# CederGroupHub/chgnet

Hardware: NVIDIA H100
Metric: structures_per_sec_EFS (higher is better)
Workload: dtype f32

## Files before the change

chgnet_b200/csrc/gated_ws.cu:

```cuda
#include "gated_common.cuh"
#include "tc.cuh"

namespace chg {
namespace gated {
namespace {

constexpr int WS_THREADS = 512;
constexpr int TR = 128;
constexpr int HALF_BYTES = TR * 64 * 4;
constexpr int IMG_BYTES = 64 * 64 * 4;
constexpr int STRIP = 16;

struct WsSmem {
  static constexpr int IMG_OFF = 0;
  static constexpr int HS_OFF = 4 * IMG_BYTES;
  static constexpr int O_OFF = HS_OFF + 2 * HALF_BYTES;
  static constexpr int GIDX_OFF = O_OFF + HALF_BYTES;
  static constexpr int EIDX_OFF = GIDX_OFF + 2 * 3 * TR * 4;
  static constexpr int B2_OFF = EIDX_OFF + 4 * TR * 4;
  static constexpr int LN_OFF = B2_OFF + 128 * 4;
  static constexpr int TOTAL = LN_OFF + 256 * 4;
};

struct WsBars {
  uint64_t a_full[2], a_empty[2];
};

struct FusedArgs {
  const float* p_a;
  const float* p_b;
  const float* p_c;
  const float* wgt;
  const int32_t* idx0;
  const int32_t* idx1;
  const int32_t* idx2;
  const int32_t* ptr;
  int32_t n_rows, n_seg;
  const float* w2t;
  const float* b2;
  const float* ln;
  float* out;
  float* parts;
  float* save_pre;
  float* save_p;
};

__device__ __forceinline__ void prefetch_l2(const void* p) { asm volatile("prefetch.global.L2 [%0];" ::"l"(p)); }
__device__ __forceinline__ int swz(int r, int c) { return r * 256 + ((c ^ (r & 7)) << 4); }

__device__ __forceinline__ void build_image_ws(uint8_t* hi, uint8_t* lo, const float* __restrict__ src, int ld, int col0,
                                               int tid) {
  for (int i = tid; i < 4096; i += (int)blockDim.x) {
    const int kk = i >> 6, n = i & 63;
    uint32_t h, l;
    tc::split_tf32(__ldg(src + (size_t)kk * ld + col0 + n), h, l);
    const uint32_t off = tc::kmajor_offset(n, kk, 64);
    *reinterpret_cast<uint32_t*>(hi + off) = h;
    *reinterpret_cast<uint32_t*>(lo + off) = l;
  }
}

__device__ __forceinline__ float quad_sum(float v) {
  v += __shfl_xor_sync(0xffffffffu, v, 1);
  v += __shfl_xor_sync(0xffffffffu, v, 2);
  return v;
}
__device__ __forceinline__ void bias_ln_frag(float (&d)[32], const float* s_b2, const float* s_gamma, const float* s_beta,
                                             bool use_ln, float* save_rows, int row0, int n_rows) {
#pragma unroll
  for (int i = 0; i < 32; ++i) d[i] += s_b2[tc::frag_col(i)];
  if (save_rows != nullptr) {
#pragma unroll
    for (int i = 0; i < 32; i += 2) {
      const int g = row0 + tc::frag_row(i);
      if (g < n_rows) *reinterpret_cast<float2*>(save_rows + (size_t)g * 128 + tc::frag_col(i)) = make_float2(d[i], d[i + 1]);
    }
  }
  if (!use_ln) return;
#pragma unroll
  for (int h = 0; h < 2; ++h) {
    float s1 = 0.f;
#pragma unroll
    for (int i = 0; i < 32; ++i)
      if (((i >> 1) & 1) == h) s1 += d[i];
    const float mean = quad_sum(s1) * (1.f / 64.f);
    float s2 = 0.f;
#pragma unroll
    for (int i = 0; i < 32; ++i)
      if (((i >> 1) & 1) == h) s2 = fmaf(d[i] - mean, d[i] - mean, s2);
    const float rstd = 1.f / sqrtf(quad_sum(s2) * (1.f / 64.f) + LN_EPS);
#pragma unroll
    for (int i = 0; i < 32; ++i)
      if (((i >> 1) & 1) == h) d[i] = fmaf((d[i] - mean) * rstd, s_gamma[tc::frag_col(i)], s_beta[tc::frag_col(i)]);
  }
}

template <int MODE>
__global__ void __launch_bounds__(WS_THREADS, 1) gated_ws_fwd_kernel(const FusedArgs a) {
  extern __shared__ __align__(1024) uint8_t smem_raw[];
  uint8_t* s_img = smem_raw + WsSmem::IMG_OFF;
  uint8_t* s_hs = smem_raw + WsSmem::HS_OFF;
  uint8_t* s_o = smem_raw + WsSmem::O_OFF;
  int* s_gidx = reinterpret_cast<int*>(smem_raw + WsSmem::GIDX_OFF);
  int* s_eidx = reinterpret_cast<int*>(smem_raw + WsSmem::EIDX_OFF);
  float* s_b2 = reinterpret_cast<float*>(smem_raw + WsSmem::B2_OFF);
  float* s_ln = reinterpret_cast<float*>(smem_raw + WsSmem::LN_OFF);
  __shared__ __align__(8) WsBars bars;

  const int tid = threadIdx.x, warp = tid >> 5, lane = tid & 31;
  const bool use_ln = a.ln != nullptr;
  const int n_tiles = (a.n_rows + TR - 1) / TR;

  build_image_ws(s_img, s_img + IMG_BYTES, a.w2t, 128, 0, tid);
  build_image_ws(s_img + 2 * IMG_BYTES, s_img + 3 * IMG_BYTES, a.w2t, 128, 64, tid);
  if (tid < 128) s_b2[tid] = a.b2[tid];
  if (tid < 256) s_ln[tid] = use_ln ? a.ln[tid] : 0.f;
  if (tid == 0) {
    for (int i = 0; i < 2; ++i) {
      tc::mbar_init(&bars.a_full[i], 128);
      tc::mbar_init(&bars.a_empty[i], 256);
    }
    tc::mbar_fence_init();
  }
  tc::fence_async_smem();
  __syncthreads();

  if (warp >= 8) {
    const int half = (warp - 8) >> 2;
    const int gt = tid - 256 - half * 128;
    const int tx = gt & 15, ty = gt >> 4;
    int* gi = s_gidx + half * 3 * TR;
    uint8_t* stage = s_hs + half * HALF_BYTES;
    const int col = half * 64 + tx * 4;
    constexpr int PB = 4;
    int tl = 0;
    for (int tile = blockIdx.x; tile < n_tiles; tile += gridDim.x, ++tl) {
      const int base = tile * TR;
      {
        const int r = min(base + gt, a.n_rows - 1);
        gi[gt] = a.idx0[r];
        gi[TR + gt] = a.idx1[r];
        gi[2 * TR + gt] = a.idx2[r];
      }
      tc::wg_barrier(1 + half, 128);
      {
        const int nt = tile + gridDim.x;
        if (nt < n_tiles) {
          const int r = min(nt * TR + gt, a.n_rows - 1);
          const float* row = MODE == BOND ? a.p_c + (size_t)r * 128 + half * 64 : a.p_b + (size_t)__ldg(a.idx2 + r) * 128 + half * 64;
          prefetch_l2(row);
          prefetch_l2(row + 32);
        }
      }
#pragma unroll 1
      for (int b = 0; b < 16 / PB; ++b) {
        float4 v[PB];
#pragma unroll
        for (int i = 0; i < PB; ++i) {
          const int row = ty + 8 * (b * PB + i);
          const float* s0 = a.p_a + (size_t)gi[row] * 256 + col;
          const float* s1 = a.p_a + (size_t)gi[TR + row] * 256 + 128 + col;
          const float* s2 = a.p_b + (size_t)gi[2 * TR + row] * 128 + col;
          v[i] = ldg4(s0) + ldg4(s1) + ldg4(s2);
          if (MODE == BOND) v[i] = v[i] + ldg4(a.p_c + (size_t)min(base + row, a.n_rows - 1) * 128 + col);
        }
        if (b == 0) tc::mbar_wait(&bars.a_empty[half], (tl & 1) ^ 1);
#pragma unroll
        for (int i = 0; i < PB; ++i) {
          const int row = ty + 8 * (b * PB + i);
          if (a.save_pre != nullptr && base + row < a.n_rows) stg4(a.save_pre + (size_t)(base + row) * 128 + col, v[i]);
          *reinterpret_cast<float4*>(stage + swz(row, tx)) =
              make_float4(silu_f(v[i].x), silu_f(v[i].y), silu_f(v[i].z), silu_f(v[i].w));
        }
      }
      tc::wg_barrier(1 + half, 128);
      tc::mbar_arrive(&bars.a_full[half]);
    }
  } else {
    const int cw = warp >> 2;
    const int t = tid & 127;
    const int row0 = cw * 64;
    int* s_seg = s_eidx;
    int* s_wrow = s_eidx + TR;
    int* s_sa = s_eidx + 2 * TR;
    int* s_sb = s_eidx + 3 * TR;
    const uint32_t img = tc::smem_u32(s_img);
    int tl = 0;
    for (int tile = blockIdx.x; tile < n_tiles; tile += gridDim.x, ++tl) {
      const int base = tile * TR;
      {
        const int r = min(base + t, a.n_rows - 1);
        if (cw == 0) {
          const int seg = a.idx0[r];
          s_seg[t] = seg;
          s_sa[t] = __ldg(a.ptr + seg);
          s_sb[t] = __ldg(a.ptr + seg + 1);
        } else {
          const int wr = MODE == BOND ? a.idx1[r] : a.idx2[r];
          s_wrow[t] = wr;
          prefetch_l2(a.wgt + (size_t)wr * 64);
          prefetch_l2(a.wgt + (size_t)wr * 64 + 32);
        }
      }
      float dc[32], dg[32];
#pragma unroll
      for (int i = 0; i < 32; ++i) dc[i] = dg[i] = 0.f;
      tc::mbar_wait(&bars.a_full[0], tl & 1);
      tc::wg_gemm_k64<64>(dc, [&](int r, int k) { return *reinterpret_cast<const float*>(s_hs + swz(row0 + r, k >> 2) + (k & 3) * 4); },
                          img, img + IMG_BYTES, 2048);
      tc::mbar_arrive(&bars.a_empty[0]);
      tc::mbar_wait(&bars.a_full[1], tl & 1);
      tc::wg_gemm_k64<64>(dg, [&](int r, int k) { return *reinterpret_cast<const float*>(s_hs + HALF_BYTES + swz(row0 + r, k >> 2) + (k & 3) * 4); },
                          img + 2 * IMG_BYTES, img + 3 * IMG_BYTES, 2048);
      tc::mbar_arrive(&bars.a_empty[1]);
      float* save = a.save_p != nullptr ? a.save_p + (size_t)base * 128 : nullptr;
      bias_ln_frag(dc, s_b2, s_ln, s_ln + 64, use_ln, save, row0, a.n_rows - base);
      bias_ln_frag(dg, s_b2 + 64, s_ln + 128, s_ln + 192, use_ln, save != nullptr ? save + 64 : nullptr, row0, a.n_rows - base);
#pragma unroll
      for (int i = 0; i < 32; i += 2) {
        const int r = row0 + tc::frag_row(i), c = tc::frag_col(i);
        *reinterpret_cast<float2*>(s_o + swz(r, c >> 2) + (c & 3) * 4) =
            make_float2(silu_f(dc[i]) * sigmoid_f(dg[i]), silu_f(dc[i + 1]) * sigmoid_f(dg[i + 1]));
      }
      tc::wg_barrier(3, 256);

      const int strip_lo = base + warp * STRIP;
      const int strip_hi = min(strip_lo + STRIP, a.n_rows);
      if (strip_lo < a.n_rows) {
        float2 w[STRIP];
#pragma unroll
        for (int i = 0; i < STRIP; ++i) {
          const int rr = warp * STRIP + i;
          const float2 w0 = __ldg(reinterpret_cast<const float2*>(a.wgt + (size_t)s_wrow[rr] * 64) + lane);
          if (MODE == ATOM) {
            w[i] = w0;
          } else {
            const float2 wi = __ldg(reinterpret_cast<const float2*>(a.wgt + (size_t)s_seg[rr] * 64) + lane);
            w[i] = make_float2(wi.x * w0.x, wi.y * w0.y);
          }
        }
        float2 acc = make_float2(0.f, 0.f);
        int cur_row = warp * STRIP;
        auto emit = [&](int row0_, const float2& v) {
          const int seg = s_seg[row0_], sa = s_sa[row0_], sb = s_sb[row0_];
          float* dst;
          if (sa >= strip_lo && sb <= strip_hi) {
            dst = a.out + (size_t)seg * 64;
          } else {
            dst = a.parts + ((size_t)(strip_lo / STRIP) * 2 + (sa < strip_lo ? 0 : 1)) * 64;
          }
          *reinterpret_cast<float2*>(dst + lane * 2) = v;
        };
#pragma unroll
        for (int i = 0; i < STRIP; ++i) {
          const int rr = warp * STRIP + i;
          if (strip_lo + i < strip_hi) {
            if (s_seg[rr] != s_seg[cur_row]) {
              emit(cur_row, acc);
              cur_row = rr;
              acc = make_float2(0.f, 0.f);
            }
            const float2 o = *reinterpret_cast<const float2*>(s_o + swz(rr, lane >> 1) + (lane & 1) * 8);
            acc.x = fmaf(o.x, w[i].x, acc.x);
            acc.y = fmaf(o.y, w[i].y, acc.y);
          }
        }
        emit(cur_row, acc);
      }
      tc::wg_barrier(3, 256);
    }
  }
}

__global__ void seg_stitch_kernel(const int32_t* __restrict__ ptr, int n_seg, const float* __restrict__ parts,
                                  float* __restrict__ out) {
  const int idx = blockIdx.x * blockDim.x + threadIdx.x;
  const int s = idx >> 4, l = idx & 15;
  if (s >= n_seg) return;
  const int a = ptr[s], b = ptr[s + 1];
  if (a >= b) {
    stg4(out + (size_t)s * 64 + l * 4, make_float4(0.f, 0.f, 0.f, 0.f));
    return;
  }
  const int k0 = a / STRIP, k1 = (b - 1) / STRIP;
  if (k0 == k1) return;
  float4 acc = ldg4(parts + ((size_t)k0 * 2 + 1) * 64 + l * 4);
  for (int k = k0 + 1; k <= k1; ++k) acc = acc + ldg4(parts + ((size_t)k * 2) * 64 + l * 4);
  stg4(out + (size_t)s * 64 + l * 4, acc);
}

template <int MODE>
int launch_fused(const FusedArgs& a, cudaStream_t stream) {
  if (a.n_seg == 0) return CHG_OK;
  if (a.n_rows > 0) {
    static bool attr_set = false;
    if (!attr_set) {
      CHG_CUDA(cudaFuncSetAttribute(gated_ws_fwd_kernel<MODE>, cudaFuncAttributeMaxDynamicSharedMemorySize, WsSmem::TOTAL));
      attr_set = true;
    }
    const int n_tiles = (a.n_rows + TR - 1) / TR;
    gated_ws_fwd_kernel<MODE><<<min(n_tiles, sm_count()), WS_THREADS, WsSmem::TOTAL, stream>>>(a);
    cudaError_t e = cudaGetLastError();
    if (e != cudaSuccess) {
      set_error("gated_ws_fwd_kernel: launch failed: %s", cudaGetErrorString(e));
      return CHG_ERR_CUDA;
    }
    count_launch();
  }
  seg_stitch_kernel<<<(a.n_seg * 16 + 255) / 256, 256, 0, stream>>>(a.ptr, a.n_seg, a.parts, a.out);
  CHG_LAUNCH_END();
}

}

int atom_conv_fused_ws(const float* pcn, const float* pe, const float* wag, const int32_t* center, const int32_t* nbr,
                       const int32_t* d2u, const int32_t* ptr_c, int n_edges, int n_atoms, const float* w2t, const float* b2,
                       const float* ln, float* agg, float* save_p, float* parts, cudaStream_t stream) {
  FusedArgs a{pcn, pe, nullptr, wag, center, nbr, d2u, ptr_c, n_edges, n_atoms, w2t, b2, ln, agg, parts, nullptr, save_p};
  return launch_fused<ATOM>(a, stream);
}

int bond_conv_fused_ws(const float* pij, const float* px, const float* pa, const float* wbg, const int32_t* ang_atom,
                       const int32_t* ang_i, const int32_t* ang_j, const int32_t* ptr_i, int n_angles, int n_slots,
                       const float* w2t, const float* b2, const float* ln, float* agg, float* save_pre, float* save_p,
                       float* parts, cudaStream_t stream) {
  FusedArgs a{pij, px, pa, wbg, ang_i, ang_j, ang_atom, ptr_i, n_angles, n_slots, w2t, b2, ln, agg, parts, save_pre, save_p};
  return launch_fused<BOND>(a, stream);
}

}
}

using namespace chg;

extern "C" int64_t chg_gated_fused_workspace_floats(int32_t n_rows) {
  if (n_rows < 0) return -1;
  const int64_t msg = (int64_t)n_rows * 64, parts = ((int64_t)n_rows + 15) / 16 * 128;
  return (msg > parts ? msg : parts) + 64;
}

extern "C" int chg_atom_conv_fused(const float* pcn, const float* pe, const float* wag, const int32_t* center,
                                   const int32_t* nbr, const int32_t* d2u, const int32_t* ptr_c, int32_t n_edges,
                                   int32_t n_atoms, const float* w2t, const float* b2, const float* ln, float* agg,
                                   float* save_p, float* work, void* stream) {
  CHG_CHECK_ARG(n_edges >= 0 && n_atoms >= 0, "negative size");
  if (n_atoms == 0) return CHG_OK;
  CHG_CHECK_ARG(ptr_c && agg, "null pointer");
  CHG_CHECK_ARG(n_edges == 0 || (pcn && pe && wag && center && nbr && d2u && w2t && b2 && work), "null pointer");
  if (gated_impl() == 3 && n_edges >= ws_min_rows())
    return gated::atom_conv_fused_ws(pcn, pe, wag, center, nbr, d2u, ptr_c, n_edges, n_atoms, w2t, b2, ln, agg, save_p, work,
                                     as_stream(stream));
  const int rc = chg_atom_conv_fwd(pcn, pe, wag, center, nbr, d2u, n_edges, w2t, b2, ln, work, save_p, nullptr, stream);
  if (rc != CHG_OK) return rc;
  return chg_segment_sum(work, 64, nullptr, ptr_c, n_atoms, n_edges, 0, agg, 64, stream);
}

extern "C" int chg_bond_conv_fused(const float* pij, const float* px, const float* pa, const float* wbg,
                                   const int32_t* ang_atom, const int32_t* ang_i, const int32_t* ang_j,
                                   const int32_t* ptr_i, int32_t n_angles, int32_t n_slots, const float* w2t,
                                   const float* b2, const float* ln, float* agg, float* save_pre, float* save_p,
                                   float* work, void* stream) {
  CHG_CHECK_ARG(n_angles >= 0 && n_slots >= 0, "negative size");
  if (n_slots == 0) return CHG_OK;
  CHG_CHECK_ARG(ptr_i && agg, "null pointer");
  CHG_CHECK_ARG(n_angles == 0 || (pij && px && pa && wbg && ang_atom && ang_i && ang_j && w2t && b2 && work), "null pointer");
  if (gated_impl() == 3 && n_angles >= ws_min_rows())
    return gated::bond_conv_fused_ws(pij, px, pa, wbg, ang_atom, ang_i, ang_j, ptr_i, n_angles, n_slots, w2t, b2, ln, agg,
                                     save_pre, save_p, work, as_stream(stream));
  const int rc = chg_bond_conv_fwd(pij, px, pa, wbg, ang_atom, ang_i, ang_j, n_angles, w2t, b2, ln, work, save_pre, save_p, stream);
  if (rc != CHG_OK) return rc;
  return chg_segment_sum(work, 64, nullptr, ptr_i, n_slots, n_angles, 0, agg, 64, stream);
}

namespace chg {
namespace gated {
namespace {

struct WsBwdSmem {
  static constexpr int IMG_OFF = 0;
  static constexpr int T1_OFF = 4 * IMG_BYTES;
  static constexpr int T2_OFF = T1_OFF + 2 * HALF_BYTES;
  static constexpr int PIDX_OFF = T2_OFF + 2 * HALF_BYTES;
  static constexpr int FIDX_OFF = PIDX_OFF + 3 * TR * 4;
  static constexpr int LN_OFF = FIDX_OFF + 3 * TR * 4;
  static constexpr int TOTAL = LN_OFF + 256 * 4;
};

struct WsBwdBars {
  uint64_t a_full, a_empty;
};

template <int MODE>
__global__ void __launch_bounds__(WS_THREADS, 1) gated_ws_bwd_kernel(const BwdArgs a) {
  extern __shared__ __align__(1024) uint8_t smem_raw[];
  uint8_t* s_img = smem_raw + WsBwdSmem::IMG_OFF;
  uint8_t* s_t1 = smem_raw + WsBwdSmem::T1_OFF;
  uint8_t* s_t2 = smem_raw + WsBwdSmem::T2_OFF;
  int* s_pidx = reinterpret_cast<int*>(smem_raw + WsBwdSmem::PIDX_OFF);
  int* s_fidx = reinterpret_cast<int*>(smem_raw + WsBwdSmem::FIDX_OFF);
  float* s_ln = reinterpret_cast<float*>(smem_raw + WsBwdSmem::LN_OFF);
  __shared__ __align__(8) WsBwdBars bars;

  const int tid = threadIdx.x, warp = tid >> 5;
  const bool use_ln = a.ln != nullptr;
  const int n_tiles = (a.n_rows + TR - 1) / TR;

  build_image_ws(s_img, s_img + IMG_BYTES, a.w2, 64, 0, tid);
  build_image_ws(s_img + 2 * IMG_BYTES, s_img + 3 * IMG_BYTES, a.w2 + 64 * 64, 64, 0, tid);
  if (tid < 256) s_ln[tid] = use_ln ? a.ln[tid] : 0.f;
  if (tid == 0) {
    tc::mbar_init(&bars.a_full, 256);
    tc::mbar_init(&bars.a_empty, 256);
    tc::mbar_fence_init();
  }
  tc::fence_async_smem();
  __syncthreads();

  if (warp < 8) {
    const int t = tid;
    const int tx = t & 15, ty = t >> 4;
    const int c0 = tx * 4;
    int tl = 0;
    for (int tile = blockIdx.x; tile < n_tiles; tile += gridDim.x, ++tl) {
      const int base = tile * TR;
      if (t < TR) {
        const int r = min(base + t, a.n_rows - 1);
        s_pidx[t] = a.idx0[r];
        s_pidx[TR + t] = a.idx1[r];
        if (MODE == ATOM) s_pidx[2 * TR + t] = a.idx2[r];
      }
      tc::wg_barrier(1, 256);
      {
        const int nt = tile + gridDim.x;
        if (nt < n_tiles) {
          const int r = min(nt * TR + (t & 127), a.n_rows - 1);
          const float* row = a.save_p + (size_t)r * 128 + (t >> 7) * 64;
          prefetch_l2(row);
          prefetch_l2(row + 32);
        }
      }
      float4 g1, g2, b1, b2v;
      if (use_ln) {
        g1 = lds4(s_ln + c0);
        b1 = lds4(s_ln + 64 + c0);
        g2 = lds4(s_ln + 128 + c0);
        b2v = lds4(s_ln + 192 + c0);
      }
      tc::mbar_wait(&bars.a_empty, (tl & 1) ^ 1);
#pragma unroll 2
      for (int pass = 0; pass < 8; ++pass) {
        const int row = pass * 16 + ty;
        const int g = base + row;
        const bool valid = g < a.n_rows;
        const int r = min(g, a.n_rows - 1);
        const float4 pc4 = ldg4(a.save_p + (size_t)r * 128 + c0);
        const float4 pg4 = ldg4(a.save_p + (size_t)r * 128 + 64 + c0);
        float4 gm, wv;
        if (MODE == ATOM) {
          gm = ldg4(a.g_in + (size_t)s_pidx[row] * 64 + c0);
          wv = ldg4(a.wgt + (size_t)s_pidx[2 * TR + row] * 64 + c0);
        } else {
          gm = ldg4(a.g_in + (size_t)s_pidx[row] * 64 + c0);
          wv = ldg4(a.wgt + (size_t)s_pidx[row] * 64 + c0);
        }
        float y1[4] = {pc4.x, pc4.y, pc4.z, pc4.w};
        float y2[4] = {pg4.x, pg4.y, pg4.z, pg4.w};
        float xh1[4], xh2[4], rstd1 = 1.f, rstd2 = 1.f;
        if (use_ln) {
          ln_stats(y1, xh1, rstd1);
          ln_stats(y2, xh2, rstd2);
#pragma unroll
          for (int j = 0; j < 4; ++j) {
            y1[j] = fmaf(xh1[j], f4at(g1, j), f4at(b1, j));
            y2[j] = fmaf(xh2[j], f4at(g2, j), f4at(b2v, j));
          }
        }
        float s1[4], core[4], gate[4];
        float4 o;
#pragma unroll
        for (int j = 0; j < 4; ++j) {
          s1[j] = sigmoid_f(y1[j]);
          core[j] = y1[j] * s1[j];
          gate[j] = sigmoid_f(y2[j]);
          f4at(o, j) = core[j] * gate[j];
        }
        float4 go;
        if (MODE == ATOM) {
          if (valid) stg4(a.g_w0 + (size_t)g * 64 + c0, gm * o);
          go = gm * wv;
        } else {
          const float4 wj = ldg4(a.wgt + (size_t)s_pidx[TR + row] * 64 + c0);
          const float4 gmo = gm * o;
          if (valid) {
            stg4(a.g_w0 + (size_t)g * 64 + c0, gmo * wj);
            stg4(a.g_w1 + (size_t)g * 64 + c0, gmo * wv);
          }
          go = gm * wv * wj;
        }
        float gy1[4], gy2[4];
#pragma unroll
        for (int j = 0; j < 4; ++j) {
          const float gj = f4at(go, j);
          gy1[j] = gj * gate[j] * (s1[j] * fmaf(y1[j], 1.f - s1[j], 1.f));
          gy2[j] = gj * core[j] * gate[j] * (1.f - gate[j]);
        }
        if (use_ln) {
          float gx[4], sa = 0.f, sb = 0.f;
#pragma unroll
          for (int j = 0; j < 4; ++j) {
            gx[j] = gy1[j] * f4at(g1, j);
            sa += gx[j];
            sb = fmaf(gx[j], xh1[j], sb);
          }
          sa = sum16(sa) * (1.f / 64.f);
          sb = sum16(sb) * (1.f / 64.f);
#pragma unroll
          for (int j = 0; j < 4; ++j) gy1[j] = rstd1 * (gx[j] - sa - xh1[j] * sb);
          sa = 0.f, sb = 0.f;
#pragma unroll
          for (int j = 0; j < 4; ++j) {
            gx[j] = gy2[j] * f4at(g2, j);
            sa += gx[j];
            sb = fmaf(gx[j], xh2[j], sb);
          }
          sa = sum16(sa) * (1.f / 64.f);
          sb = sum16(sb) * (1.f / 64.f);
#pragma unroll
          for (int j = 0; j < 4; ++j) gy2[j] = rstd2 * (gx[j] - sa - xh2[j] * sb);
        }
        *reinterpret_cast<float4*>(s_t1 + swz(row, tx)) = make_float4(gy1[0], gy1[1], gy1[2], gy1[3]);
        *reinterpret_cast<float4*>(s_t1 + HALF_BYTES + swz(row, tx)) = make_float4(gy2[0], gy2[1], gy2[2], gy2[3]);
      }
      tc::wg_barrier(1, 256);
      tc::mbar_arrive(&bars.a_full);
    }
  } else {
    const int t = tid - 256;
    const int tx = t & 15, ty = t >> 4;
    const int c0 = tx * 4;
    const int crow = t & 127, chalf = t >> 7;
    const int row0 = ((warp - 8) >> 2) * 64;
    const uint32_t img = tc::smem_u32(s_img);
    int tl = 0;
    for (int tile = blockIdx.x; tile < n_tiles; tile += gridDim.x, ++tl) {
      const int base = tile * TR;
      if (MODE == ATOM && t < TR) {
        const int r = min(base + t, a.n_rows - 1);
        s_fidx[t] = a.idx0[r];
        s_fidx[TR + t] = a.idx1[r];
        s_fidx[2 * TR + t] = a.idx2[r];
      }
      {
        const int r = min(base + crow, a.n_rows - 1);
        const float* row = MODE == ATOM ? a.p_b + (size_t)__ldg(a.idx2 + r) * 128 + chalf * 64 : a.save_pre + (size_t)r * 128 + chalf * 64;
        prefetch_l2(row);
        prefetch_l2(row + 32);
      }
      tc::mbar_wait(&bars.a_full, tl & 1);
#pragma unroll 1
      for (int half = 0; half < 2; ++half) {
        float d[32];
#pragma unroll
        for (int i = 0; i < 32; ++i) d[i] = 0.f;
        const uint8_t* src = s_t1 + half * HALF_BYTES;
        tc::wg_gemm_k64<64>(d, [&](int r, int k) { return *reinterpret_cast<const float*>(src + swz(row0 + r, k >> 2) + (k & 3) * 4); },
                            img + half * 2 * IMG_BYTES, img + (half * 2 + 1) * IMG_BYTES, 2048);
        uint8_t* dst = s_t2 + half * HALF_BYTES;
#pragma unroll
        for (int i = 0; i < 32; i += 2) {
          const int r = row0 + tc::frag_row(i), c = tc::frag_col(i);
          *reinterpret_cast<float2*>(dst + swz(r, c >> 2) + (c & 3) * 4) = make_float2(d[i], d[i + 1]);
        }
      }
      tc::mbar_arrive(&bars.a_empty);
      tc::wg_barrier(2, 256);
#pragma unroll 2
      for (int pass = 0; pass < 8; ++pass) {
        const int row = pass * 16 + ty;
        const int g = base + row;
        float4 vc, vg;
        if (MODE == ATOM) {
          const float* s0 = a.p_a + (size_t)s_fidx[row] * 256 + c0;
          const float* s1 = a.p_a + (size_t)s_fidx[TR + row] * 256 + 128 + c0;
          const float* s2 = a.p_b + (size_t)s_fidx[2 * TR + row] * 128 + c0;
          vc = ldg4(s0) + ldg4(s1) + ldg4(s2);
          vg = ldg4(s0 + 64) + ldg4(s1 + 64) + ldg4(s2 + 64);
        } else {
          const int r = min(g, a.n_rows - 1);
          vc = ldg4(a.save_pre + (size_t)r * 128 + c0);
          vg = ldg4(a.save_pre + (size_t)r * 128 + 64 + c0);
        }
        const float4 hc = *reinterpret_cast<const float4*>(s_t2 + swz(row, tx));
        const float4 hg = *reinterpret_cast<const float4*>(s_t2 + HALF_BYTES + swz(row, tx));
        if (g < a.n_rows) {
          stg4(a.g_pre + (size_t)g * 128 + c0,
               make_float4(hc.x * dsilu_f(vc.x), hc.y * dsilu_f(vc.y), hc.z * dsilu_f(vc.z), hc.w * dsilu_f(vc.w)));
          stg4(a.g_pre + (size_t)g * 128 + 64 + c0,
               make_float4(hg.x * dsilu_f(vg.x), hg.y * dsilu_f(vg.y), hg.z * dsilu_f(vg.z), hg.w * dsilu_f(vg.w)));
        }
      }
      tc::wg_barrier(2, 256);
    }
  }
}

template <int MODE>
int launch_ws_bwd(const BwdArgs& a, cudaStream_t stream) {
  if (a.n_rows == 0) return CHG_OK;
  static bool attr_set = false;
  if (!attr_set) {
    CHG_CUDA(cudaFuncSetAttribute(gated_ws_bwd_kernel<MODE>, cudaFuncAttributeMaxDynamicSharedMemorySize, WsBwdSmem::TOTAL));
    attr_set = true;
  }
  const int n_tiles = (a.n_rows + TR - 1) / TR;
  gated_ws_bwd_kernel<MODE><<<min(n_tiles, sm_count()), WS_THREADS, WsBwdSmem::TOTAL, stream>>>(a);
  CHG_LAUNCH_END();
}

}

int atom_conv_bwd_ws(const BwdArgs& a, cudaStream_t stream) { return launch_ws_bwd<ATOM>(a, stream); }
int bond_conv_bwd_ws(const BwdArgs& a, cudaStream_t stream) { return launch_ws_bwd<BOND>(a, stream); }

}
}
```

Measured before the change: 10910.

## Add L2 eviction-policy hints, bulk prefetches, and split backward empty barrier

```diff
diff --git a/chgnet_b200/csrc/gated_ws.cu b/chgnet_b200/csrc/gated_ws.cu
--- a/chgnet_b200/csrc/gated_ws.cu
+++ b/chgnet_b200/csrc/gated_ws.cu
@@ -46,6 +46,45 @@
 };
 
 __device__ __forceinline__ void prefetch_l2(const void* p) { asm volatile("prefetch.global.L2 [%0];" ::"l"(p)); }
+
+__device__ __forceinline__ uint64_t l2_evict_first() {
+  uint64_t p;
+  asm volatile("createpolicy.fractional.L2::evict_first.b64 %0, 1.0;" : "=l"(p));
+  return p;
+}
+__device__ __forceinline__ uint64_t l2_evict_last() {
+  uint64_t p;
+  asm volatile("createpolicy.fractional.L2::evict_last.b64 %0, 1.0;" : "=l"(p));
+  return p;
+}
+__device__ __forceinline__ float4 ldg4_stream(const float* p, uint64_t pol) {
+  float4 v;
+  asm("ld.global.nc.L1::no_allocate.L2::cache_hint.v4.f32 {%0, %1, %2, %3}, [%4], %5;"
+      : "=f"(v.x), "=f"(v.y), "=f"(v.z), "=f"(v.w) : "l"(p), "l"(pol));
+  return v;
+}
+__device__ __forceinline__ float4 ldg4_table(const float* p, uint64_t pol) {
+  float4 v;
+  asm("ld.global.nc.L2::cache_hint.v4.f32 {%0, %1, %2, %3}, [%4], %5;"
+      : "=f"(v.x), "=f"(v.y), "=f"(v.z), "=f"(v.w) : "l"(p), "l"(pol));
+  return v;
+}
+__device__ __forceinline__ float2 ldg2_table(const float* p, uint64_t pol) {
+  float2 v;
+  asm("ld.global.nc.L2::cache_hint.v2.f32 {%0, %1}, [%2], %3;" : "=f"(v.x), "=f"(v.y) : "l"(p), "l"(pol));
+  return v;
+}
+__device__ __forceinline__ void stg4_stream(float* p, const float4& v, uint64_t pol) {
+  asm volatile("st.global.L2::cache_hint.v4.f32 [%0], {%1, %2, %3, %4}, %5;" ::"l"(p), "f"(v.x), "f"(v.y), "f"(v.z), "f"(v.w),
+               "l"(pol)
+               : "memory");
+}
+__device__ __forceinline__ void stg2_stream(float* p, const float2& v, uint64_t pol) {
+  asm volatile("st.global.L2::cache_hint.v2.f32 [%0], {%1, %2}, %3;" ::"l"(p), "f"(v.x), "f"(v.y), "l"(pol) : "memory");
+}
+__device__ __forceinline__ void prefetch_half_row(const float* p, uint64_t pol) {
+  asm volatile("cp.async.bulk.prefetch.L2.global.L2::cache_hint [%0], 256, %1;" ::"l"(p), "l"(pol) : "memory");
+}
 __device__ __forceinline__ int swz(int r, int c) { return r * 256 + ((c ^ (r & 7)) << 4); }
 
 __device__ __forceinline__ void build_image_ws(uint8_t* hi, uint8_t* lo, const float* __restrict__ src, int ld, int col0,
@@ -66,14 +105,14 @@
   return v;
 }
 __device__ __forceinline__ void bias_ln_frag(float (&d)[32], const float* s_b2, const float* s_gamma, const float* s_beta,
-                                             bool use_ln, float* save_rows, int row0, int n_rows) {
+                                             bool use_ln, float* save_rows, int row0, int n_rows, uint64_t pol_stream) {
 #pragma unroll
   for (int i = 0; i < 32; ++i) d[i] += s_b2[tc::frag_col(i)];
   if (save_rows != nullptr) {
 #pragma unroll
     for (int i = 0; i < 32; i += 2) {
       const int g = row0 + tc::frag_row(i);
-      if (g < n_rows) *reinterpret_cast<float2*>(save_rows + (size_t)g * 128 + tc::frag_col(i)) = make_float2(d[i], d[i + 1]);
+      if (g < n_rows) stg2_stream(save_rows + (size_t)g * 128 + tc::frag_col(i), make_float2(d[i], d[i + 1]), pol_stream);
     }
   }
   if (!use_ln) return;
@@ -133,6 +172,7 @@
     uint8_t* stage = s_hs + half * HALF_BYTES;
     const int col = half * 64 + tx * 4;
     constexpr int PB = 4;
+    const uint64_t pol_stream = l2_evict_first(), pol_table = l2_evict_last();
     int tl = 0;
     for (int tile = blockIdx.x; tile < n_tiles; tile += gridDim.x, ++tl) {
       const int base = tile * TR;
@@ -147,9 +187,8 @@
         const int nt = tile + gridDim.x;
         if (nt < n_tiles) {
           const int r = min(nt * TR + gt, a.n_rows - 1);
-          const float* row = MODE == BOND ? a.p_c + (size_t)r * 128 + half * 64 : a.p_b + (size_t)__ldg(a.idx2 + r) * 128 + half * 64;
-          prefetch_l2(row);
-          prefetch_l2(row + 32);
+          if (MODE == BOND) prefetch_half_row(a.p_c + (size_t)r * 128 + half * 64, pol_stream);
+          else prefetch_half_row(a.p_b + (size_t)__ldg(a.idx2 + r) * 128 + half * 64, pol_table);
         }
       }
 #pragma unroll 1
@@ -161,14 +200,14 @@
           const float* s0 = a.p_a + (size_t)gi[row] * 256 + col;
           const float* s1 = a.p_a + (size_t)gi[TR + row] * 256 + 128 + col;
           const float* s2 = a.p_b + (size_t)gi[2 * TR + row] * 128 + col;
-          v[i] = ldg4(s0) + ldg4(s1) + ldg4(s2);
-          if (MODE == BOND) v[i] = v[i] + ldg4(a.p_c + (size_t)min(base + row, a.n_rows - 1) * 128 + col);
+          v[i] = ldg4_table(s0, pol_table) + ldg4_table(s1, pol_table) + ldg4_table(s2, pol_table);
+          if (MODE == BOND) v[i] = v[i] + ldg4_stream(a.p_c + (size_t)min(base + row, a.n_rows - 1) * 128 + col, pol_stream);
         }
         if (b == 0) tc::mbar_wait(&bars.a_empty[half], (tl & 1) ^ 1);
 #pragma unroll
         for (int i = 0; i < PB; ++i) {
           const int row = ty + 8 * (b * PB + i);
-          if (a.save_pre != nullptr && base + row < a.n_rows) stg4(a.save_pre + (size_t)(base + row) * 128 + col, v[i]);
+          if (a.save_pre != nullptr && base + row < a.n_rows) stg4_stream(a.save_pre + (size_t)(base + row) * 128 + col, v[i], pol_stream);
           *reinterpret_cast<float4*>(stage + swz(row, tx)) =
               make_float4(silu_f(v[i].x), silu_f(v[i].y), silu_f(v[i].z), silu_f(v[i].w));
         }
@@ -198,8 +237,7 @@
         } else {
           const int wr = MODE == BOND ? a.idx1[r] : a.idx2[r];
           s_wrow[t] = wr;
-          prefetch_l2(a.wgt + (size_t)wr * 64);
-          prefetch_l2(a.wgt + (size_t)wr * 64 + 32);
+          prefetch_half_row(a.wgt + (size_t)wr * 64, l2_evict_last());
         }
       }
       float dc[32], dg[32];
@@ -214,8 +252,10 @@
                           img + 2 * IMG_BYTES, img + 3 * IMG_BYTES, 2048);
       tc::mbar_arrive(&bars.a_empty[1]);
       float* save = a.save_p != nullptr ? a.save_p + (size_t)base * 128 : nullptr;
-      bias_ln_frag(dc, s_b2, s_ln, s_ln + 64, use_ln, save, row0, a.n_rows - base);
-      bias_ln_frag(dg, s_b2 + 64, s_ln + 128, s_ln + 192, use_ln, save != nullptr ? save + 64 : nullptr, row0, a.n_rows - base);
+      const uint64_t pol_stream = l2_evict_first();
+      bias_ln_frag(dc, s_b2, s_ln, s_ln + 64, use_ln, save, row0, a.n_rows - base, pol_stream);
+      bias_ln_frag(dg, s_b2 + 64, s_ln + 128, s_ln + 192, use_ln, save != nullptr ? save + 64 : nullptr, row0, a.n_rows - base,
+                   pol_stream);
 #pragma unroll
       for (int i = 0; i < 32; i += 2) {
         const int r = row0 + tc::frag_row(i), c = tc::frag_col(i);
@@ -227,15 +267,16 @@
       const int strip_lo = base + warp * STRIP;
       const int strip_hi = min(strip_lo + STRIP, a.n_rows);
       if (strip_lo < a.n_rows) {
+        const uint64_t pol_table = l2_evict_last();
         float2 w[STRIP];
 #pragma unroll
         for (int i = 0; i < STRIP; ++i) {
           const int rr = warp * STRIP + i;
-          const float2 w0 = __ldg(reinterpret_cast<const float2*>(a.wgt + (size_t)s_wrow[rr] * 64) + lane);
+          const float2 w0 = ldg2_table(a.wgt + (size_t)s_wrow[rr] * 64 + lane * 2, pol_table);
           if (MODE == ATOM) {
             w[i] = w0;
           } else {
-            const float2 wi = __ldg(reinterpret_cast<const float2*>(a.wgt + (size_t)s_seg[rr] * 64) + lane);
+            const float2 wi = ldg2_table(a.wgt + (size_t)s_seg[rr] * 64 + lane * 2, pol_table);
             w[i] = make_float2(wi.x * w0.x, wi.y * w0.y);
           }
         }
@@ -387,7 +428,7 @@
 };
 
 struct WsBwdBars {
-  uint64_t a_full, a_empty;
+  uint64_t a_full, a_empty[2];
 };
 
 template <int MODE>
@@ -410,7 +451,8 @@
   if (tid < 256) s_ln[tid] = use_ln ? a.ln[tid] : 0.f;
   if (tid == 0) {
     tc::mbar_init(&bars.a_full, 256);
-    tc::mbar_init(&bars.a_empty, 256);
+    tc::mbar_init(&bars.a_empty[0], 256);
+    tc::mbar_init(&bars.a_empty[1], 256);
     tc::mbar_fence_init();
   }
   tc::fence_async_smem();
@@ -420,9 +462,11 @@
     const int t = tid;
     const int tx = t & 15, ty = t >> 4;
     const int c0 = tx * 4;
+    const uint64_t pol_stream = l2_evict_first(), pol_table = l2_evict_last();
     int tl = 0;
     for (int tile = blockIdx.x; tile < n_tiles; tile += gridDim.x, ++tl) {
       const int base = tile * TR;
+      const int nt = tile + gridDim.x;
       if (t < TR) {
         const int r = min(base + t, a.n_rows - 1);
         s_pidx[t] = a.idx0[r];
@@ -430,15 +474,7 @@
         if (MODE == ATOM) s_pidx[2 * TR + t] = a.idx2[r];
       }
       tc::wg_barrier(1, 256);
-      {
-        const int nt = tile + gridDim.x;
-        if (nt < n_tiles) {
-          const int r = min(nt * TR + (t & 127), a.n_rows - 1);
-          const float* row = a.save_p + (size_t)r * 128 + (t >> 7) * 64;
-          prefetch_l2(row);
-          prefetch_l2(row + 32);
-        }
-      }
+      if (nt < n_tiles) prefetch_half_row(a.save_p + (size_t)min(nt * TR + (t & 127), a.n_rows - 1) * 128 + (t >> 7) * 64, pol_stream);
       float4 g1, g2, b1, b2v;
       if (use_ln) {
         g1 = lds4(s_ln + c0);
@@ -446,22 +482,21 @@
         g2 = lds4(s_ln + 128 + c0);
         b2v = lds4(s_ln + 192 + c0);
       }
-      tc::mbar_wait(&bars.a_empty, (tl & 1) ^ 1);
 #pragma unroll 2
       for (int pass = 0; pass < 8; ++pass) {
         const int row = pass * 16 + ty;
         const int g = base + row;
         const bool valid = g < a.n_rows;
         const int r = min(g, a.n_rows - 1);
-        const float4 pc4 = ldg4(a.save_p + (size_t)r * 128 + c0);
-        const float4 pg4 = ldg4(a.save_p + (size_t)r * 128 + 64 + c0);
+        const float4 pc4 = ldg4_stream(a.save_p + (size_t)r * 128 + c0, pol_stream);
+        const float4 pg4 = ldg4_stream(a.save_p + (size_t)r * 128 + 64 + c0, pol_stream);
         float4 gm, wv;
         if (MODE == ATOM) {
-          gm = ldg4(a.g_in + (size_t)s_pidx[row] * 64 + c0);
-          wv = ldg4(a.wgt + (size_t)s_pidx[2 * TR + row] * 64 + c0);
+          gm = ldg4_table(a.g_in + (size_t)s_pidx[row] * 64 + c0, pol_table);
+          wv = ldg4_table(a.wgt + (size_t)s_pidx[2 * TR + row] * 64 + c0, pol_table);
         } else {
-          gm = ldg4(a.g_in + (size_t)s_pidx[row] * 64 + c0);
-          wv = ldg4(a.wgt + (size_t)s_pidx[row] * 64 + c0);
+          gm = ldg4_table(a.g_in + (size_t)s_pidx[row] * 64 + c0, pol_table);
+          wv = ldg4_table(a.wgt + (size_t)s_pidx[row] * 64 + c0, pol_table);
         }
         float y1[4] = {pc4.x, pc4.y, pc4.z, pc4.w};
         float y2[4] = {pg4.x, pg4.y, pg4.z, pg4.w};
@@ -486,14 +521,14 @@
         }
         float4 go;
         if (MODE == ATOM) {
-          if (valid) stg4(a.g_w0 + (size_t)g * 64 + c0, gm * o);
+          if (valid) stg4_stream(a.g_w0 + (size_t)g * 64 + c0, gm * o, pol_stream);
           go = gm * wv;
         } else {
-          const float4 wj = ldg4(a.wgt + (size_t)s_pidx[TR + row] * 64 + c0);
+          const float4 wj = ldg4_table(a.wgt + (size_t)s_pidx[TR + row] * 64 + c0, pol_table);
           const float4 gmo = gm * o;
           if (valid) {
-            stg4(a.g_w0 + (size_t)g * 64 + c0, gmo * wj);
-            stg4(a.g_w1 + (size_t)g * 64 + c0, gmo * wv);
+            stg4_stream(a.g_w0 + (size_t)g * 64 + c0, gmo * wj, pol_stream);
+            stg4_stream(a.g_w1 + (size_t)g * 64 + c0, gmo * wv, pol_stream);
           }
           go = gm * wv * wj;
         }
@@ -528,7 +563,9 @@
 #pragma unroll
           for (int j = 0; j < 4; ++j) gy2[j] = rstd2 * (gx[j] - sa - xh2[j] * sb);
         }
+        if (pass == 0) tc::mbar_wait(&bars.a_empty[0], (tl & 1) ^ 1);
         *reinterpret_cast<float4*>(s_t1 + swz(row, tx)) = make_float4(gy1[0], gy1[1], gy1[2], gy1[3]);
+        if (pass == 0) tc::mbar_wait(&bars.a_empty[1], (tl & 1) ^ 1);
         *reinterpret_cast<float4*>(s_t1 + HALF_BYTES + swz(row, tx)) = make_float4(gy2[0], gy2[1], gy2[2], gy2[3]);
       }
       tc::wg_barrier(1, 256);
@@ -541,6 +578,7 @@
     const int crow = t & 127, chalf = t >> 7;
     const int row0 = ((warp - 8) >> 2) * 64;
     const uint32_t img = tc::smem_u32(s_img);
+    const uint64_t pol_stream = l2_evict_first(), pol_table = l2_evict_last();
     int tl = 0;
     for (int tile = blockIdx.x; tile < n_tiles; tile += gridDim.x, ++tl) {
       const int base = tile * TR;
@@ -552,9 +590,8 @@
       }
       {
         const int r = min(base + crow, a.n_rows - 1);
-        const float* row = MODE == ATOM ? a.p_b + (size_t)__ldg(a.idx2 + r) * 128 + chalf * 64 : a.save_pre + (size_t)r * 128 + chalf * 64;
-        prefetch_l2(row);
-        prefetch_l2(row + 32);
+        if (MODE == ATOM) prefetch_half_row(a.p_b + (size_t)__ldg(a.idx2 + r) * 128 + chalf * 64, pol_table);
+        else prefetch_half_row(a.save_pre + (size_t)r * 128 + chalf * 64, pol_stream);
       }
       tc::mbar_wait(&bars.a_full, tl & 1);
 #pragma unroll 1
@@ -565,6 +602,7 @@
         const uint8_t* src = s_t1 + half * HALF_BYTES;
         tc::wg_gemm_k64<64>(d, [&](int r, int k) { return *reinterpret_cast<const float*>(src + swz(row0 + r, k >> 2) + (k & 3) * 4); },
                             img + half * 2 * IMG_BYTES, img + (half * 2 + 1) * IMG_BYTES, 2048);
+        tc::mbar_arrive(&bars.a_empty[half]);
         uint8_t* dst = s_t2 + half * HALF_BYTES;
 #pragma unroll
         for (int i = 0; i < 32; i += 2) {
@@ -572,7 +610,6 @@
           *reinterpret_cast<float2*>(dst + swz(r, c >> 2) + (c & 3) * 4) = make_float2(d[i], d[i + 1]);
         }
       }
-      tc::mbar_arrive(&bars.a_empty);
       tc::wg_barrier(2, 256);
 #pragma unroll 2
       for (int pass = 0; pass < 8; ++pass) {
@@ -583,20 +620,20 @@
           const float* s0 = a.p_a + (size_t)s_fidx[row] * 256 + c0;
           const float* s1 = a.p_a + (size_t)s_fidx[TR + row] * 256 + 128 + c0;
           const float* s2 = a.p_b + (size_t)s_fidx[2 * TR + row] * 128 + c0;
-          vc = ldg4(s0) + ldg4(s1) + ldg4(s2);
-          vg = ldg4(s0 + 64) + ldg4(s1 + 64) + ldg4(s2 + 64);
+          vc = ldg4_table(s0, pol_table) + ldg4_table(s1, pol_table) + ldg4_table(s2, pol_table);
+          vg = ldg4_table(s0 + 64, pol_table) + ldg4_table(s1 + 64, pol_table) + ldg4_table(s2 + 64, pol_table);
         } else {
           const int r = min(g, a.n_rows - 1);
-          vc = ldg4(a.save_pre + (size_t)r * 128 + c0);
-          vg = ldg4(a.save_pre + (size_t)r * 128 + 64 + c0);
+          vc = ldg4_stream(a.save_pre + (size_t)r * 128 + c0, pol_stream);
+          vg = ldg4_stream(a.save_pre + (size_t)r * 128 + 64 + c0, pol_stream);
         }
         const float4 hc = *reinterpret_cast<const float4*>(s_t2 + swz(row, tx));
         const float4 hg = *reinterpret_cast<const float4*>(s_t2 + HALF_BYTES + swz(row, tx));
         if (g < a.n_rows) {
-          stg4(a.g_pre + (size_t)g * 128 + c0,
-               make_float4(hc.x * dsilu_f(vc.x), hc.y * dsilu_f(vc.y), hc.z * dsilu_f(vc.z), hc.w * dsilu_f(vc.w)));
-          stg4(a.g_pre + (size_t)g * 128 + 64 + c0,
-               make_float4(hg.x * dsilu_f(vg.x), hg.y * dsilu_f(vg.y), hg.z * dsilu_f(vg.z), hg.w * dsilu_f(vg.w)));
+          stg4_stream(a.g_pre + (size_t)g * 128 + c0,
+                      make_float4(hc.x * dsilu_f(vc.x), hc.y * dsilu_f(vc.y), hc.z * dsilu_f(vc.z), hc.w * dsilu_f(vc.w)), pol_stream);
+          stg4_stream(a.g_pre + (size_t)g * 128 + 64 + c0,
+                      make_float4(hg.x * dsilu_f(vg.x), hg.y * dsilu_f(vg.y), hg.z * dsilu_f(vg.z), hg.w * dsilu_f(vg.w)), pol_stream);
         }
       }
       tc::wg_barrier(2, 256);
```

Result: faster. 11140, median of 6 (+2.2%).
